# chreisinger/ViLGOD

Hardware: AMD Instinct MI355X
Metric: pseudo-labeled LiDAR frames/sec (150k pts, ~60 clusters) (higher is better)
Workload: dtype f16

## Files before the change

vilgod_amd/csrc/dev/vit_dev_entry.inc:

```
int vg_gemm_variant(int var, const void* d_X, const void* d_Wt, const float* d_bias, void* d_C, int M, int N, int K, int ldc, void* stream) {
    if (M % GBM || N % GBN || K % GK) return VG_ERR_ARG;
    int nwg = (M / GBM) * (N / GBN);
    hipStream_t st = (hipStream_t)stream;
#define VG_VAR(V)                                                                                                          \
    case V:                                                                                                                \
        (void)hipFuncSetAttribute((const void*)k_gemm_f16<EPI_BIAS, V>, hipFuncAttributeMaxDynamicSharedMemorySize, G_LDS_BYTES); \
        hipLaunchKernelGGL((k_gemm_f16<EPI_BIAS, V>), dim3(nwg), dim3(512), G_LDS_BYTES, st, (const f16*)d_X, (const f16*)d_Wt, \
                           d_bias, d_C, nullptr, M, N, K, ldc, gemm_chunk_tiles(N, K));                                   \
        break;
    switch (var) { VG_VAR(0) VG_VAR(1) VG_VAR(2) VG_VAR(3)
        case 20: return launch_gemm_pp<EPI_BIAS, 4, false>(d_X, d_Wt, d_bias, d_C, nullptr, M, N, K, ldc, st, nullptr);
        case 21: return launch_gemm_pp<EPI_BIAS, 5, false>(d_X, d_Wt, d_bias, d_C, nullptr, M, N, K, ldc, st, nullptr);
        case 22: return launch_gemm_pp<EPI_BIAS, 4, false, 1>(d_X, d_Wt, d_bias, d_C, nullptr, M, N, K, ldc, st, nullptr);
        case 23: return launch_gemm_pp<EPI_BIAS, 5, false, 1>(d_X, d_Wt, d_bias, d_C, nullptr, M, N, K, ldc, st, nullptr);
        case 30: return launch_gemm_pp16<EPI_BIAS, 4>(d_X, d_Wt, d_bias, d_C, nullptr, M, N, K, ldc, st);
        case 32: return launch_gemm_pp64<EPI_BIAS>(d_X, d_Wt, d_bias, d_C, nullptr, M, N, K, ldc, st);
        case 36: return launch_gemm_pp64<EPI_BIAS, false, true>(d_X, d_Wt, d_bias, d_C, nullptr, M, N, K, ldc, st);
        default: return VG_ERR_ARG; }
#undef VG_VAR
    VG_LAUNCH_CHECK();
    return VG_OK;
}

int vg_gemm_ln_consumer(int epi, const void* d_X, const void* d_Wt, const float* d_bias, const float* d_c1, const void* d_stats,
                        void* d_C, int M, int N, int K, void* stream) {
    hipStream_t st = (hipStream_t)stream;
    if (epi == 0) return launch_gemm_pp64<EPI_BIAS, false, false, 1>(d_X, d_Wt, d_bias, d_C, nullptr, M, N, K, N, st, nullptr, d_c1, (LnPartial*)d_stats);
    if (epi == 1) return launch_gemm_pp64<EPI_BIAS_GELU, false, false, 1>(d_X, d_Wt, d_bias, d_C, nullptr, M, N, K, N, st, nullptr, d_c1, (LnPartial*)d_stats);
    return VG_ERR_ARG;
}

int vg_gemm_trace(int var, const void* d_X, const void* d_Wt, const float* d_bias, void* d_C, int64_t* d_trace, int M, int N,
                  int K, int ldc, void* stream) {
    hipStream_t st = (hipStream_t)stream;
    switch (var) {
        case 20: return launch_gemm_pp<EPI_BIAS, 4, true>(d_X, d_Wt, d_bias, d_C, nullptr, M, N, K, ldc, st, (long long*)d_trace);
        case 21: return launch_gemm_pp<EPI_BIAS, 5, true>(d_X, d_Wt, d_bias, d_C, nullptr, M, N, K, ldc, st, (long long*)d_trace);
        case 22: return launch_gemm_pp<EPI_BIAS, 4, true, 1>(d_X, d_Wt, d_bias, d_C, nullptr, M, N, K, ldc, st, (long long*)d_trace);
        case 23: return launch_gemm_pp<EPI_BIAS, 5, true, 1>(d_X, d_Wt, d_bias, d_C, nullptr, M, N, K, ldc, st, (long long*)d_trace);
        case 32: return launch_gemm_pp64<EPI_BIAS, true>(d_X, d_Wt, d_bias, d_C, nullptr, M, N, K, ldc, st, (long long*)d_trace);
        case 33: return launch_gemm_pp64<EPI_BIAS_GELU, true>(d_X, d_Wt, d_bias, d_C, nullptr, M, N, K, ldc, st, (long long*)d_trace);
        case 34: return launch_gemm_pp64<EPI_BIAS_RESID, true>(d_X, d_Wt, d_bias, nullptr, (float*)d_C, M, N, K, ldc, st, (long long*)d_trace);
        case 35: return launch_gemm_pp64<EPI_BIAS_RESID_H, true>(d_X, d_Wt, d_bias, nullptr, (float*)d_C, M, N, K, ldc, st, (long long*)d_trace);
        case 50: return launch_gemm_w4<EPI_BIAS, 0, VG_W4_TRACE_VAR>(d_X, d_Wt, d_bias, d_C, nullptr, M, N, K, ldc, st, nullptr, nullptr, nullptr, (long long*)d_trace);
        case 40: return launch_gemm_x2<EPI_BIAS, 0, true>(d_X, d_Wt, d_bias, d_C, nullptr, M, N, K, ldc, st, nullptr, nullptr, nullptr, (long long*)d_trace);
        default: return VG_ERR_ARG; }
    VG_LAUNCH_CHECK();
    return VG_OK;
}

int vg_attention_trace(const void* d_qkv, void* d_out, int n_crops, int T, int W, int heads, int ld, int64_t* d_trace, void* stream) {
    if (!d_qkv || !d_out || n_crops <= 0 || T > AT_MAXT || heads * 64 != W) return VG_ERR_ARG;
    const int items = n_crops * heads;
    hipStream_t st = (hipStream_t)stream;
    if (d_trace) return launch_attention<true>((const f16*)d_qkv, (f16*)d_out, T, W, heads, ld, items, (long long*)d_trace, st);
    return launch_attention<false>((const f16*)d_qkv, (f16*)d_out, T, W, heads, ld, items, nullptr, st);
}
```

vilgod_amd/csrc/vit.hip:

```cpp
#include "common.h"
#include <hip/hip_fp16.h>
#include <string.h>
#include <stdlib.h>
#include <string>
#include <vector>
#include <map>
#include <atomic>
#include <mutex>
#include <utility>

typedef _Float16 f16;
typedef f16 f16x8 __attribute__((ext_vector_type(8)));
typedef f16 f16x4 __attribute__((ext_vector_type(4)));
typedef float f32x16 __attribute__((ext_vector_type(16)));

#define QGELU_C (-1.702f * 1.4426950408889634f)
enum { EPI_BIAS = 0, EPI_BIAS_GELU = 1, EPI_BIAS_RESID = 2, EPI_NONE_F32 = 3,
       EPI_BIAS_RESID_H = 4,
       EPI_BIAS_RESID_HL = 5 };

__device__ __forceinline__ int xcd_remap(int bid, int nwg) {
    int q = nwg >> 3, r = nwg & 7, xcd = bid & 7, s = bid >> 3;
    int base = (xcd < r) ? xcd * (q + 1) : r * (q + 1) + (xcd - r) * q;
    return base + s;
// ... 599 lines not shown
    float sum = 0.f;
    const int tail = T - 32 * (nkb - 1);
#pragma unroll
    for (int kb = 0; kb < 7; ++kb) {
        if (kb < nkb) {
#pragma unroll
            for (int g = 0; g < 4; ++g) {
                if (kb < nkb - 1 || 8 * g < tail) {
#pragma unroll
                    for (int r = 4 * g; r < 4 * g + 4; ++r) {
                        const float p = __builtin_amdgcn_exp2f(fmaf(sacc[kb][r], c2, mc));
                        sacc[kb][r] = p;
                        sum += p;
                    }
                } else {
#pragma unroll
                    for (int r = 4 * g; r < 4 * g + 4; ++r) sacc[kb][r] = 0.f;
                }
            }
        }
    }
    sum += __shfl_xor(sum, 32);
    const float inv = 1.0f / sum;
    AT_STAMP(4)

    f32x16 oacc[2];
#pragma unroll
    for (int dt = 0; dt < 2; ++dt)
#pragma unroll
        for (int r = 0; r < 16; ++r) oacc[dt][r] = 0.f;
#pragma unroll
    for (int kb = 0; kb < 7; ++kb) {
        if (kb < nkb) {
#pragma unroll
            for (int s = 0; s < 2; ++s) {
                if (kb == nkb - 1 && 16 * s >= tail) continue;
                f16x8 pf;
#pragma unroll
                for (int j = 0; j < 8; ++j) pf[j] = (f16)sacc[kb][8 * s + j];
#pragma unroll
                for (int dt = 0; dt < 2; ++dt) {
                    f16x4 lo, hi;
                    if (TR) {
                        const char* vb = (const char*)Vs + tr_off + ((kb * 32 + 16 * s) * AT_KLD + dt * 32) * 2;
                        lo = __builtin_bit_cast(f16x4, __builtin_amdgcn_ds_read_tr16_b64_v4i16((__attribute__((address_space(3))) s16x4v*)vb));
                        hi = __builtin_bit_cast(f16x4, __builtin_amdgcn_ds_read_tr16_b64_v4i16((__attribute__((address_space(3))) s16x4v*)(vb + 8 * AT_KLD * 2)));
                    } else {
                        const f16* vp = Vt + (dt * 32 + r31) * AT_VLD + kb * 32 + 16 * s + 4 * hh;
                        lo = *(const f16x4*)vp; hi = *(const f16x4*)(vp + 8);
                    }
                    f16x8 vf = {lo[0], lo[1], lo[2], lo[3], hi[0], hi[1], hi[2], hi[3]};
                    oacc[dt] = __builtin_amdgcn_mfma_f32_32x32x16_f16(vf, pf, oacc[dt], 0, 0, 0);
                }
            }
        }
    }
    AT_STAMP(5)
#pragma unroll
    for (int dt = 0; dt < 2; ++dt)
#pragma unroll
        for (int g = 0; g < 4; ++g) {
            f16x4 h4;
#pragma unroll
            for (int e = 0; e < 4; ++e) h4[e] = (f16)(oacc[dt][4 * g + e] * inv);
            *(f16x4*)(Qs + r31 * AT_KLD + dt * 32 + 8 * g + 4 * hh) = h4;
        }
#pragma unroll
    for (int it = 0; it < 4; ++it) {
        const int qr = q0 + it * 8 + crow;
        const f16x8 v = *(const f16x8*)(Qs + (it * 8 + crow) * AT_KLD + cpart * 8);
        if (qr < T) *(f16x8*)(obase + ooff[it]) = v;
    }
    }
    AT_STAMP(6)
    __syncthreads();
    AT_STAMP(7)
    }
    if (TRACE && trace && lane == 0) {
        long long* o = trace + ((size_t)blockIdx.x * 7 + wave) * 8;
#pragma unroll
        for (int i = 0; i < 8; ++i) o[i] = tr[i];
    }
#undef AT_STAMP
}

#define AL_MAXT 1024
#define AL_KB 64
#define AL_BUF (AL_KB * AT_KLD)
#define AL_LDS_BYTES ((4 * AL_BUF + 4 * 32 * AT_KLD) * 2)
__global__ __launch_bounds__(256, 2) void k_attention_f16_long(const f16* __restrict__ qkv, f16* __restrict__ out, int T, int W,
                                                               int heads, int ld, int n_items, int q_tiles) {
    extern __shared__ __attribute__((aligned(16))) char al_smem[];
    f16* const KV = (f16*)al_smem;
    const int tid = threadIdx.x, lane = tid & 63, wave = tid >> 6;
    f16* const Os = KV + 4 * AL_BUF + wave * 32 * AT_KLD;
    const int r31 = lane & 31, hh = lane >> 5;
    const int crow = lane >> 3, cpart = lane & 7;
    const int tr_i = lane & 15, tr_g = lane >> 4;
    const int tr_off = ((4 * (tr_g >> 1) + (tr_i >> 2)) * AT_KLD + 16 * (tr_g & 1) + 4 * (tr_i & 3)) * 2;
    const int ntile = (T + 31) / 32;
    const int qt = q_tiles < ntile ? q_tiles : ntile;
    const int npass = (qt + 3) / 4;
    const int nkb = (T + AL_KB - 1) / AL_KB;
    const int per_item = npass * nkb;
    const int my_items = (int)blockIdx.x < n_items ? (n_items - 1 - (int)blockIdx.x) / (int)gridDim.x + 1 : 0;
    const int nsteps = my_items * per_item;
    if (nsteps == 0) return;
    auto decode = [&](int s, int& item, int& pass, int& kb) {
        const int u = s / per_item, r = s - u * per_item;
        item = (int)blockIdx.x + u * (int)gridDim.x;
        pass = r / nkb;
        kb = r - pass * nkb;
    };
    uint4 kreg[2];
    f16x8 vreg[2], qn[4];
    auto fetch = [&](int s) {
        int item, pass, kb;
        decode(s, item, pass, kb);
        const int crop = item / heads, head = item - crop * heads;
        const f16* base = qkv + (size_t)crop * T * ld + head * 64;
#pragma unroll
        for (int it = 0; it < 2; ++it) {
            const int c = tid + it * 256, key = kb * AL_KB + (c >> 3), part = c & 7;
            const unsigned off = (unsigned)((key < T ? key : T - 1) * ld + part * 8);
            kreg[it] = *(const uint4*)(base + W + off);
            vreg[it] = *(const f16x8*)(base + 2 * W + off);
        }
        if (kb == 0) {
            const int qr = (pass * 4 + wave) * 32 + r31;
            const unsigned off = (unsigned)((qr < T ? qr : T - 1) * ld + hh * 8);
#pragma unroll
            for (int s4 = 0; s4 < 4; ++s4) qn[s4] = *(const f16x8*)(base + off + s4 * 16);
        }
    };
    auto stage = [&](int s) {
        int item, pass, kb;
        decode(s, item, pass, kb);
        f16* const Kb = KV + (s & 1) * 2 * AL_BUF;
        f16* const Vb = Kb + AL_BUF;
        const f16x8 z = {0, 0, 0, 0, 0, 0, 0, 0};
#pragma unroll
        for (int it = 0; it < 2; ++it) {
            const int c = tid + it * 256, row = c >> 3, part = c & 7;
            const bool live = kb * AL_KB + row < T;
            *(uint4*)(Kb + row * AT_KLD + part * 8) = live ? kreg[it] : make_uint4(0, 0, 0, 0);
            *(f16x8*)(Vb + row * AT_KLD + part * 8) = live ? vreg[it] : z;
        }
    };
    fetch(0);
    stage(0);
    __syncthreads();
    const float c2 = 0.125f * 1.4426950408889634f;
    f16x8 qf[4];
    f32x16 oacc[2];
    float m = -INFINITY, l = 0.f;
    for (int s = 0; s < nsteps; ++s) {
        int item, pass, kb;
        decode(s, item, pass, kb);
        if (kb == 0) {
#pragma unroll
            for (int s4 = 0; s4 < 4; ++s4) qf[s4] = qn[s4];
#pragma unroll
            for (int dt = 0; dt < 2; ++dt)
#pragma unroll
                for (int r = 0; r < 16; ++r) oacc[dt][r] = 0.f;
            m = -INFINITY;
// ... 175 lines not shown
    }
}

template <typename TI>
__global__ __launch_bounds__(256) void k_head(const TI* __restrict__ x, const float* __restrict__ lw,
                                              const float* __restrict__ lb, const float* __restrict__ proj,
                                              float* __restrict__ feat, int T, int W, int D) {
    extern __shared__ float sm[];
    __shared__ float red[8];
    const int crop = blockIdx.x, tid = threadIdx.x, lane = tid & 63, wave = tid >> 6;
    const TI* src = x + (size_t)crop * T * W;
    float s = 0.f;
    for (int c = tid; c < W; c += 256) s += (float)src[c];
    s = vg_wave_sum(s);
    if (lane == 0) red[wave] = s;
    __syncthreads();
    float mean = (red[0] + red[1] + red[2] + red[3]) / (float)W;
    __syncthreads();
    float q = 0.f;
    for (int c = tid; c < W; c += 256) {
        float d = (float)src[c] - mean;
        q += d * d;
    }
    q = vg_wave_sum(q);
    if (lane == 0) red[wave] = q;
    __syncthreads();
    float rstd = rsqrtf((red[0] + red[1] + red[2] + red[3]) / (float)W + 1e-5f);
    for (int c = tid; c < W; c += 256) sm[c] = ((float)src[c] - mean) * rstd * lw[c] + lb[c];
    __syncthreads();
    for (int j = tid; j < D; j += 256) {
        float a = 0.f;
#pragma unroll 16
        for (int i = 0; i < W; ++i)
            a = fmaf(sm[i], proj[(size_t)i * D + j], a);
        feat[(size_t)crop * D + j] = a;
    }
}

__global__ __launch_bounds__(64) void k_clip_scores(const float* __restrict__ feat, const float* __restrict__ text,
                                                    float* __restrict__ probs, int* __restrict__ top1,
                                                    float* __restrict__ top1_score, int n, int D, int Kc) {
    const int crop = blockIdx.x, lane = threadIdx.x;
    const float* f = feat + (size_t)crop * D;
    float ss = 0.f;
    for (int i = lane; i < D; i += 64) ss += f[i] * f[i];
    float nrm = sqrtf(vg_wave_sum(ss));
    float logit = -INFINITY;
    if (lane < Kc) {
        float a = 0.f;
        for (int i = 0; i < D; ++i) a = fmaf(100.0f * (f[i] / nrm), text[(size_t)lane * D + i], a);
        logit = a;
    }
    float mx = vg_wave_max(logit);
    float e = (lane < Kc) ? expf(logit - mx) : 0.f;
    float p = e / vg_wave_sum(e);
    if (lane < Kc) probs[(size_t)crop * Kc + lane] = p;
    float best = (lane < Kc) ? p : -1.f;
    int bi = lane;
#pragma unroll
    for (int o = 32; o > 0; o >>= 1) {
        float ob = __shfl_xor(best, o);
        int oi = __shfl_xor(bi, o);
        if (ob > best || (ob == best && oi < bi)) {
            best = ob;
            bi = oi;
        }
    }
    if (lane == 0) {
        top1[crop] = bi;
        top1_score[crop] = best;
    }
}

#define VG_PROF_MAX 4096
struct vg_vit {
    int width, layers, heads, patch, res, out_dim, dtype, T;
#ifdef VG_DEV
    bool gemm_x2 = getenv("VG_GEMM_X2") ? atoi(getenv("VG_GEMM_X2")) != 0 : false;
#endif
    bool cls_last = !(getenv("VG_VIT_CLS_LAST") && atoi(getenv("VG_VIT_CLS_LAST")) == 0);
    int splitk_max = getenv("VG_GEMM_SPLITK") ? atoi(getenv("VG_GEMM_SPLITK")) : 0;
    bool att_tr = !(getenv("VG_ATT_TR") && atoi(getenv("VG_ATT_TR")) == 0);
    bool att_stagger = !(getenv("VG_ATT_STAGGER") && atoi(getenv("VG_ATT_STAGGER")) == 0);
    bool f32_mfma = !(getenv("VG_GEMM_F32_MFMA") && atoi(getenv("VG_GEMM_F32_MFMA")) == 0);
    int gemm_w4 = getenv("VG_GEMM_W4") ? atoi(getenv("VG_GEMM_W4")) : 1;
    int n_cu = 0;
    bool resid_hl = false;
    bool resid_h = false;
    int prof_on = 0, prof_n = 0;
    hipEvent_t prof_ev[2 * VG_PROF_MAX];
    double prof_flops[VG_PROF_MAX];
    int prof_kind[VG_PROF_MAX];
    bool prof_init = false;
    std::map<std::string, void*> w;
    std::map<std::string, size_t> numel;
    bool ln_fold = false;
    std::atomic<bool> fold_ready{false}, warmed{false};
    float in_mean[3] = {0.48145466f, 0.4578275f, 0.40821073f}, in_std[3] = {0.26862954f, 0.26130258f, 0.27577711f};
    std::atomic<bool> conv1_ready{false};
    std::atomic<uint64_t> weights_gen{0};
    std::mutex mtx;
    std::map<std::string, void*> w32;
};

static bool is_gemm_weight(const std::string& n) {
    return n == "conv1.weight" || n.find("in_proj_weight") != std::string::npos ||
           n.find("out_proj.weight") != std::string::npos || n.find("c_fc.weight") != std::string::npos ||
           n.find("c_proj.weight") != std::string::npos;
}

static int vit_kpad(const vg_vit* v) { return (3 * v->patch * v->patch + 63) / 64 * 64; }

static int gemm_chunk_tiles(int N, int K) {
    const int ntn = N / GBN;
#ifdef VG_DEV
    if (getenv("VG_GEMM_NO_CHUNK")) return ntn;
#endif
    const long tile_bytes = (long)GBN * K * 2;
    int cw_max = (int)(2400000L / tile_bytes);
    if (cw_max < 1) cw_max = 1;
    if (cw_max >= ntn) return ntn;
    int nchunks = (ntn + cw_max - 1) / cw_max;
    while (ntn % nchunks) ++nchunks;
    return ntn / nchunks;
}

typedef float f32x4 __attribute__((ext_vector_type(4)));
#ifdef VG_DEV
#include "dev/vit_gemm_pp16.inc"
#endif

struct LnPartial { float mean, m2; };
__device__ __forceinline__ float row256_sum(float v) {
    v += __builtin_bit_cast(float, __builtin_amdgcn_update_dpp(0, __builtin_bit_cast(int, v), 0xB1, 0xF, 0xF, true));
    v += __builtin_bit_cast(float, __builtin_amdgcn_update_dpp(0, __builtin_bit_cast(int, v), 0x4E, 0xF, 0xF, true));
    v += __builtin_bit_cast(float, __builtin_amdgcn_update_dpp(0, __builtin_bit_cast(int, v), 0x141, 0xF, 0xF, true));
    v += __builtin_bit_cast(float, __builtin_amdgcn_update_dpp(0, __builtin_bit_cast(int, v), 0x140, 0xF, 0xF, true));
    const int b = __builtin_bit_cast(int, v);
    return (__builtin_bit_cast(float, __builtin_amdgcn_readlane(b, 0)) + __builtin_bit_cast(float, __builtin_amdgcn_readlane(b, 16))) +
           (__builtin_bit_cast(float, __builtin_amdgcn_readlane(b, 32)) + __builtin_bit_cast(float, __builtin_amdgcn_readlane(b, 48)));
}

template <int EPI, bool TRACE = false, bool PERSIST = false, int LN = 0, bool SPLITK = false>
__global__ __launch_bounds__(512, 1) void k_gemm_f16_pp64(const f16* __restrict__ X, const f16* __restrict__ Wt,
                                                          const float* __restrict__ bias, void* __restrict__ Cout,
                                                          float* __restrict__ resid, int M, int N, int K, int ldc, int cw,
                                                          long long* __restrict__ trace = nullptr,
                                                          const float* __restrict__ ln_c1 = nullptr, LnPartial* __restrict__ ln_stats = nullptr,
                                                          f16* __restrict__ ln_x16 = nullptr, int sk_parts = 1) {
    static_assert(!SPLITK || (EPI == EPI_NONE_F32 && !PERSIST && LN == 0), "split-K partials are raw fp32 tiles");
    constexpr int BM = 256, BN = 256, NT = 512, TM = 8, TN = 4;
    constexpr int XBUF = 32768, WBASE = 2 * XBUF, WBUF = 32768;
    extern __shared__ __attribute__((aligned(16))) char smem[];
    const int tid = threadIdx.x, wave = __builtin_amdgcn_readfirstlane(tid >> 6);
    const int ntm = M / BM;
    const int grp = wave >> 2, wn = wave & 3;
    long long tr_entry = 0, tr_load = 0, tr_bar = 0, tr_mma = 0, tr_wait = 0, tr_t0 = 0, tr_w0 = 0, tr_main = 0, tr_w_entry = 0;
    if (TRACE) { tr_entry = clock64(); tr_w_entry = wall_clock64(); }
    const int nt_all = ntm * (N / BN);
    const int xq = nt_all >> 3, xr_ = nt_all & 7, xcd = blockIdx.x & 7;
    const int xbase = (xcd < xr_) ? xcd * (xq + 1) : xr_ * (xq + 1) + (xcd - xr_) * xq;
    const int xcnt = xq + (xcd < xr_ ? 1 : 0);
    for (int ti = PERSIST ? (int)(blockIdx.x >> 3) : 0; ti < (PERSIST ? xcnt : 1); ti += PERSIST ? (int)(gridDim.x >> 3) : 1) {
    int lane = tid & 63;
    if (PERSIST) asm volatile("" : "+v"(lane));
    const int t = PERSIST ? xbase + ti : xcd_remap(blockIdx.x, gridDim.x);
// ... 774 lines not shown
        int dev = 0;
        (void)hipGetDevice(&dev);
        (void)hipDeviceGetAttribute(&v->n_cu, hipDeviceAttributeMultiprocessorCount, dev);
    }
    const bool prof = v->prof_on && v->prof_n < VG_PROF_MAX;
    if (prof) (void)hipEventRecord(v->prof_ev[2 * v->prof_n], st);
    struct Closer {
        vg_vit* v; bool prof; hipStream_t st; double fl; int kind;
        ~Closer() {
            if (prof) {
                (void)hipEventRecord(v->prof_ev[2 * v->prof_n + 1], st);
                v->prof_kind[v->prof_n] = kind;
                v->prof_flops[v->prof_n++] = fl;
            }
        }
    } closer{v, prof, st, 2.0 * (double)M * (double)N * (double)K, use_pp ? 1 : 0};
    if constexpr (EPI == EPI_BIAS_RESID_HL) {
        if (!(LN == 2 && v->dtype == 1 && v->gemm_w4 && use_pp && M % 256 == 0 && K % 64 == 0 && K / 64 >= 4 && resid && ln_x16)) return VG_ERR_ARG;
        return launch_gemm_w4<EPI, LN>(X, Wt, bias, C, resid, M, N, K, ldc, st, ln_c1, ln_stats, ln_x16);
    } else
    if constexpr (EPI == EPI_BIAS_RESID_H) {
        if (!(use_pp && K % 64 == 0 && K / 64 >= 2)) return VG_ERR_ARG;
        return launch_gemm_pp64<EPI>(X, Wt, bias, C, resid, M, N, K, ldc, st);
    } else
    if (v->dtype == 1) {
        if (M % GBM || N % GBN || K % GK) return VG_ERR_ARG;
        if (use_pp) {
            {
#ifdef VG_DEV
                static const int persist_mask = getenv("VG_GEMM_PERSIST") ? atoi(getenv("VG_GEMM_PERSIST")) : 0;
                if constexpr (LN == 0 && (EPI == EPI_BIAS || EPI == EPI_BIAS_GELU || EPI == EPI_BIAS_RESID)) {
                    if ((persist_mask >> EPI) & 1) return launch_gemm_pp64<EPI, false, true>(X, Wt, bias, C, resid, M, N, K, ldc, st);
                }
#endif
#ifdef VG_DEV
                if (v->gemm_x2 && K % 256 == 0 && (LN != 1 || K / 64 <= X2_LN_MAXP))
                    return launch_gemm_x2<EPI, LN>(X, Wt, bias, C, resid, M, N, K, ldc, st, ln_c1, ln_stats, ln_x16);
                if (v->gemm_x2 && LN != 0) return VG_ERR_ARG;
#endif
                if constexpr (EPI == EPI_BIAS_RESID && LN != 1) {
                    if (sk_scratch && M % 256 == 0 && !(v->gemm_w4 && K / 64 >= 4)) {
                        const SplitPlan sp = splitk_plan(M / 256, N / 256, K / 64, sk_bytes, v->splitk_max, v->n_cu);
                        if (sp.parts) {
                            const int rc = launch_gemm_pp64<EPI, false, false, LN>(X, Wt, bias, C, resid, sp.r_main * 256, N, K, ldc, st, nullptr, ln_c1, ln_stats, ln_x16);
                            if (rc) return rc;
                            return launch_gemm_resid_tail<LN>(X, Wt, bias, resid, sp.r_main * 256, M - sp.r_main * 256, N, K, ldc, sp.parts, sk_scratch, st,
                                                              ln_stats, ln_x16);
                        }
                    }
                }
                if (v->gemm_w4 && K / 64 >= 4) {
#ifdef VG_DEV
                    if constexpr (LN == 0 && EPI == EPI_BIAS) {
                        switch (v->gemm_w4) { VG_W4_DEV_CASES(EPI, LN) }
                    }
#endif
                    return launch_gemm_w4<EPI, LN>(X, Wt, bias, C, resid, M, N, K, ldc, st, ln_c1, ln_stats, ln_x16);
                }
                return launch_gemm_pp64<EPI, false, false, LN>(X, Wt, bias, C, resid, M, N, K, ldc, st, nullptr, ln_c1, ln_stats, ln_x16);
            }
        }
        if (LN != 0) return VG_ERR_ARG;
        int nwg = (M / GBM) * (N / GBN);
        VG_MAX_DYNAMIC_LDS(k_gemm_f16<EPI>, G_LDS_BYTES);
        hipLaunchKernelGGL((k_gemm_f16<EPI>), dim3(nwg), dim3(512), G_LDS_BYTES, st, (const f16*)X, (const f16*)Wt, bias, C,
                           resid, M, N, K, ldc, gemm_chunk_tiles(N, K));
    } else {
        if (M % 64 || N % 64 || K % 16) return VG_ERR_ARG;
        if (M % 128 == 0 && N % 128 == 0 && v->f32_mfma) {
            hipLaunchKernelGGL((k_gemm_f32_mfma<EPI>), dim3((M / 128) * (N / 128)), dim3(256), 0, st, (const float*)X, (const float*)Wt, bias,
                               (float*)C, resid, M, N, K);
        } else {
            int nwg = (M / 64) * (N / 64);
            hipLaunchKernelGGL((k_gemm_f32<EPI>), dim3(nwg), dim3(256), 0, st, (const float*)X, (const float*)Wt, bias,
                               (float*)C, resid, M, N, K);
        }
    }
    VG_LAUNCH_CHECK();
    return VG_OK;
}

template <bool TRACE>
static int launch_attention(const f16* qkv, f16* out, int T, int W, int heads, int ld, int items, long long* trace, hipStream_t st,
                            int q_tiles = 7, bool tr = true, bool stagger = true) {
    if (T > AT_MAXT && !TRACE) {
        if (T > AL_MAXT) return VG_ERR_ARG;
        static std::atomic<int> n_cu_{0};
        int n_cu = n_cu_.load();
        if (!n_cu) { int dev = 0; (void)hipGetDevice(&dev); (void)hipDeviceGetAttribute(&n_cu, hipDeviceAttributeMultiprocessorCount, dev); if (n_cu < 8) n_cu = 256; n_cu_.store(n_cu); }
        const dim3 grid(items < 2 * n_cu ? items : 2 * n_cu);
        VG_MAX_DYNAMIC_LDS(k_attention_f16_long, AL_LDS_BYTES);
        hipLaunchKernelGGL(k_attention_f16_long, grid, dim3(256), AL_LDS_BYTES, st, qkv, out, T, W, heads, ld, items, q_tiles);
        VG_LAUNCH_CHECK();
        return VG_OK;
    }
    const int nkb = (T + 31) / 32;
    if (nkb < 1 || nkb > 7) return VG_ERR_ARG;
    if (T == 197 && !TRACE && tr && stagger) {
        const dim3 grid7(items < 256 ? items : 256);
        VG_MAX_DYNAMIC_LDS((k_attention_f16<false, 7, 197, true, true>), AT_LDS_BYTES_TR);
        hipLaunchKernelGGL((k_attention_f16<false, 7, 197, true, true>), grid7, dim3(448), AT_LDS_BYTES_TR, st, qkv, out, T, W, heads, ld, items, trace, q_tiles);
        VG_LAUNCH_CHECK();
        return VG_OK;
    }
    if (T == 197 && !TRACE && tr) {
        const dim3 grid7(items < 256 ? items : 256);
        VG_MAX_DYNAMIC_LDS((k_attention_f16<false, 7, 197, true>), AT_LDS_BYTES_TR);
        hipLaunchKernelGGL((k_attention_f16<false, 7, 197, true>), grid7, dim3(448), AT_LDS_BYTES_TR, st, qkv, out, T, W, heads, ld, items, trace, q_tiles);
        VG_LAUNCH_CHECK();
        return VG_OK;
    }
    const dim3 grid(items < 256 ? items : 256), block(448);
#define VG_ATT(N)                                                                                                                  \
    case N: {                                                                                                                      \
        VG_MAX_DYNAMIC_LDS((k_attention_f16<TRACE, N>), AT_LDS_BYTES);                                                              \
        hipLaunchKernelGGL((k_attention_f16<TRACE, N>), grid, block, AT_LDS_BYTES, st, qkv, out, T, W, heads, ld, items, trace, q_tiles);   \
        break; }
    if (T == 197 && !TRACE) {
        VG_MAX_DYNAMIC_LDS((k_attention_f16<false, 7, 197>), AT_LDS_BYTES);
        hipLaunchKernelGGL((k_attention_f16<false, 7, 197>), grid, block, AT_LDS_BYTES, st, qkv, out, T, W, heads, ld, items, trace, q_tiles);
        VG_LAUNCH_CHECK();
        return VG_OK;
    }
    switch (nkb) { VG_ATT(1) VG_ATT(2) VG_ATT(3) VG_ATT(4) VG_ATT(5) VG_ATT(6) VG_ATT(7) }
#undef VG_ATT
    VG_LAUNCH_CHECK();
    return VG_OK;
}

__global__ __launch_bounds__(256) void k_ln_fold(const float* __restrict__ W32, const float* __restrict__ g, const float* __restrict__ beta,
                                                 const float* __restrict__ b, f16* __restrict__ Wf, float* __restrict__ c1,
                                                 float* __restrict__ c2, int K) {
    __shared__ double sh1[256], sh2[256];
    const int n = blockIdx.x, tid = threadIdx.x;
    double s1 = 0.0, s2 = 0.0;
    for (int k = tid; k < K; k += 256) {
        const float w = W32[(size_t)n * K + k];
        const f16 wf = (f16)(g[k] * w);
        Wf[(size_t)n * K + k] = wf;
        s1 += (double)(float)wf;
        s2 += (double)beta[k] * (double)w;
    }
    sh1[tid] = s1; sh2[tid] = s2;
    __syncthreads();
    for (int o = 128; o > 0; o >>= 1) {
        if (tid < o) { sh1[tid] += sh1[tid + o]; sh2[tid] += sh2[tid + o]; }
        __syncthreads();
    }
    if (tid == 0) { c1[n] = (float)sh1[0]; c2[n] = (float)((double)b[n] + sh2[0]); }
}

static void* vit_w(const vg_vit* v, const std::string& n) {
    auto it = v->w.find(n);
    return it == v->w.end() ? nullptr : it->second;
}

static int vit_fold_ln(vg_vit* v, hipStream_t st) {
    if (!v->ln_fold || v->fold_ready.load()) return VG_OK;
    std::lock_guard<std::mutex> lock(v->mtx);
    if (v->fold_ready.load()) return VG_OK;
    const int W = v->width;
    for (int l = 0; l < v->layers; ++l) {
        const std::string p = "transformer.resblocks." + std::to_string(l) + ".";
        const char* sets[2][4] = {{"ln_1.weight", "ln_1.bias", "attn.in_proj_weight", "attn.in_proj_bias"},
                                  {"ln_2.weight", "ln_2.bias", "mlp.c_fc.weight", "mlp.c_fc.bias"}};
        for (int k = 0; k < 2; ++k) {
            const std::string wn = p + sets[k][2];
            auto it32 = v->w32.find(wn);
            const float* g = (const float*)vit_w(v, p + sets[k][0]);
            const float* be = (const float*)vit_w(v, p + sets[k][1]);
            const float* b = (const float*)vit_w(v, p + sets[k][3]);
            if (it32 == v->w32.end() || !g || !be || !b) continue;
            const int N = (int)(v->numel[wn] / (size_t)W);
            for (const char* suffix : {"#ln", "#c1", "#c2"}) {
                auto old = v->w.find(wn + suffix);
                if (old != v->w.end()) { (void)hipFree(old->second); v->w.erase(old); }
            }
            void *wf = nullptr, *c1 = nullptr, *c2 = nullptr;
            VG_CHECK(hipMalloc(&wf, (size_t)N * W * 2));
            VG_CHECK(hipMalloc(&c1, (size_t)N * 4));
// ... 249 lines not shown
    const float* pos_tab = (const float*)need(input_kind == 3 ? "positional_embedding#1ch" : "positional_embedding");
    int rc = input_kind == 3 ? launch_gemm<EPI_NONE_F32>(v, patches, need("conv1.weight#1ch"), nullptr, pe, nullptr, (int)Pp, W, v->patch * v->patch, st)
                             : launch_gemm<EPI_NONE_F32>(v, patches, need("conv1.weight"), nullptr, pe, nullptr, (int)Pp, W, (int)Kp, st);
    if (rc) return rc;
    if (!pos_tab) return VG_ERR_ARG;
    const bool rh = v->resid_h;
    bool ln1_done = false;
    f16* xh = (f16*)x;
    const int64_t Mc = pad128(n_crops);
    const bool cls_fits = Mc * W * 16 + Mc * (W / 64) * 8 <= Mp * (3 * W + 256) * es;
    const bool hl = v->resid_hl && fold && !rh && v->dtype == 1 && L > 1 && W % 256 == 0 && cls_fits;
    f16* xlo = (f16*)x;
    if (rh)
        hipLaunchKernelGGL((k_embed_lnpre<f16>), dim3((unsigned)((Mp + 3) / 4)), dim3(256), 0, st, pe, (const float*)need("class_embedding"),
                           pos_tab, (const float*)need("ln_pre.weight"),
                           (const float*)need("ln_pre.bias"), xh, (int)M, T, W, (int)Mp);
    else {
        ln1_done = v->dtype == 1 && L > 0;
        const float* lw1 = ln1_done ? (const float*)need("transformer.resblocks.0.ln_1.weight") : nullptr;
        const float* lb1 = ln1_done ? (const float*)need("transformer.resblocks.0.ln_1.bias") : nullptr;
        if (ln1_done && (!lw1 || !lb1)) return VG_ERR_ARG;
        hipLaunchKernelGGL((k_embed_lnpre<float>), dim3((unsigned)((Mp + 3) / 4)), dim3(256), 0, st, pe, (const float*)need("class_embedding"),
                           pos_tab, (const float*)need("ln_pre.weight"),
                           (const float*)need("ln_pre.bias"), x, (int)M, T, W, (int)Mp, lw1, lb1, ln1_done ? (f16*)h : (f16*)nullptr,
                           hl ? (f16*)x16 : (f16*)nullptr, hl ? xlo : (f16*)nullptr);
    }
    VG_LAUNCH_CHECK();
    for (int l = 0; l < L; ++l) {
        std::string p = "transformer.resblocks." + std::to_string(l) + ".";
        const char* names[] = {"ln_1.weight", "ln_1.bias", "attn.in_proj_weight", "attn.in_proj_bias", "attn.out_proj.weight",
                               "attn.out_proj.bias", "ln_2.weight", "ln_2.bias", "mlp.c_fc.weight", "mlp.c_fc.bias",
                               "mlp.c_proj.weight", "mlp.c_proj.bias"};
        void* wp[12];
        for (int i = 0; i < 12; ++i) {
            wp[i] = need(p + names[i]);
            if (!wp[i]) {
                fprintf(stderr, "[vilgod_hip] vg_vit_encode: weight %s%s not set\n", p.c_str(), names[i]);
                return VG_ERR_ARG;
            }
        }
        void *fw1 = nullptr, *fw2 = nullptr;
        const float *f1c1 = nullptr, *f1c2 = nullptr, *f2c1 = nullptr, *f2c2 = nullptr;
        if (fold) {
            fw1 = need(p + "attn.in_proj_weight#ln"); f1c1 = (const float*)need(p + "attn.in_proj_weight#c1"); f1c2 = (const float*)need(p + "attn.in_proj_weight#c2");
            fw2 = need(p + "mlp.c_fc.weight#ln");     f2c1 = (const float*)need(p + "mlp.c_fc.weight#c1");     f2c2 = (const float*)need(p + "mlp.c_fc.weight#c2");
            if (!fw1 || !f1c1 || !f1c2 || !fw2 || !f2c1 || !f2c2) return VG_ERR_ARG;
        }
        if (l == 0 && ln1_done) {
        } else if (fold) {
        } else if (rh)
            hipLaunchKernelGGL((k_layernorm<f16, f16>), dim3((unsigned)((M + 3) / 4)), dim3(256), 0, st, (const f16*)xh, (const float*)wp[0], (const float*)wp[1], (f16*)h, (int)M, W, 1);
        else if (v->dtype == 1)
            hipLaunchKernelGGL((k_layernorm<f16>), dim3((unsigned)((M + 3) / 4)), dim3(256), 0, st, x, (const float*)wp[0], (const float*)wp[1], (f16*)h, (int)M, W, 1);
        else
            hipLaunchKernelGGL((k_layernorm<float>), dim3((unsigned)((M + 3) / 4)), dim3(256), 0, st, x, (const float*)wp[0], (const float*)wp[1], (float*)h, (int)M, W, 1);
        VG_LAUNCH_CHECK();
        const bool cls_only = v->cls_last && fold && !rh && l == L - 1 && L > 1 && cls_fits;
        if (hl && l == L - 1 && !cls_only) return VG_ERR_ARG;
        if (cls_only && W % 256 == 0) {
            const int nst = v->gemm_w4 ? W >> 7 : W >> 8;
            char* cb = (char*)mlp;
            f16* x16q = (f16*)cb;              cb += Mc * W * 2;
            f16* qc = (f16*)cb;                cb += Mc * W * 2;
            LnPartial* lnq = (LnPartial*)cb;
            rc = launch_gemm<EPI_BIAS, 1>(v, x16, (const f16*)fw1 + (size_t)W * W, f1c2 + W, (f16*)qkv + W, nullptr, (int)Mp, 2 * W, W, st, qkv_ld,
                                          f1c1 + W, lnst);
            if (rc) return rc;
            hipLaunchKernelGGL(k_gather_cls_ln, dim3((unsigned)Mc), dim3(256), 0, st, (const f16*)x16, (const LnPartial*)lnst, x16q, lnq, n_crops, T, W, nst);
            VG_LAUNCH_CHECK();
            rc = launch_gemm<EPI_BIAS, 1>(v, x16q, fw1, f1c2, qc, nullptr, (int)Mc, W, W, st, 0, f1c1, lnq);
            if (rc) return rc;
            hipLaunchKernelGGL(k_scatter_cls_q, dim3((unsigned)n_crops), dim3(256), 0, st, (const f16*)qc, (f16*)qkv, T, W, qkv_ld);
            VG_LAUNCH_CHECK();
        } else
        if (fold && !(l == 0 && ln1_done))
            rc = launch_gemm<EPI_BIAS, 1>(v, x16, fw1, f1c2, qkv, nullptr, (int)Mp, 3 * W, W, st, qkv_ld, f1c1, lnst);
        else
            rc = launch_gemm<EPI_BIAS>(v, h, wp[2], (const float*)wp[3], qkv, nullptr, (int)Mp, 3 * W, W, st, qkv_ld);
        if (rc) return rc;
        if (v->dtype == 1) {
            {
                const bool aprof = v->prof_on && v->prof_n < VG_PROF_MAX;
                if (aprof) (void)hipEventRecord(v->prof_ev[2 * v->prof_n], st);
                rc = launch_attention<false>((const f16*)qkv, (f16*)h, T, W, H, qkv_ld, n_crops * H, nullptr, st, cls_only ? 1 : (T + 31) / 32, v->att_tr, v->att_stagger);
                if (rc) return rc;
                if (aprof) {
                    (void)hipEventRecord(v->prof_ev[2 * v->prof_n + 1], st);
                    v->prof_kind[v->prof_n] = cls_only ? 3 : 2;
                    v->prof_flops[v->prof_n++] = 4.0 * (cls_only ? 1.0 : (double)T) * (double)T * 64.0 * (double)(n_crops * H);
                }
            }
        } else {
            size_t lds = ((size_t)T * 65 + (size_t)T * 64 + 16 * (size_t)T) * sizeof(float);
            static bool attr = false;
            if (!attr) {
                VG_CHECK(hipFuncSetAttribute((const void*)k_attention_f32, hipFuncAttributeMaxDynamicSharedMemorySize, 160 * 1024));
                attr = true;
            }
            hipLaunchKernelGGL(k_attention_f32, dim3(n_crops * H), dim3(256), lds, st, (const float*)qkv, (float*)h, T, W, H);
        }
        VG_LAUNCH_CHECK();
        if (cls_only) {
            char* cb = (char*)qkv;
            float* xc = (float*)cb;            cb += Mc * W * 4;
            f16* hc = (f16*)cb;                cb += Mc * W * 2;
            f16* x16c = (f16*)cb;              cb += Mc * W * 2;
            f16* mlpc = (f16*)cb;              cb += Mc * 4 * W * 2;
            LnPartial* lnc = (LnPartial*)cb;
            hipLaunchKernelGGL(k_gather_cls, dim3((unsigned)Mc), dim3(256), 0, st, (const f16*)h, (const float*)x, hc, xc, n_crops, T, W,
                               hl ? (const f16*)x16 : (const f16*)nullptr, hl ? (const f16*)xlo : (const f16*)nullptr);
            VG_LAUNCH_CHECK();
            rc = launch_gemm<EPI_BIAS_RESID, 2>(v, hc, wp[4], (const float*)wp[5], nullptr, xc, (int)Mc, W, W, st, 0, nullptr, lnc, x16c);
            if (rc) return rc;
            rc = launch_gemm<EPI_BIAS_GELU, 1>(v, x16c, fw2, f2c2, mlpc, nullptr, (int)Mc, 4 * W, W, st, 0, f2c1, lnc);
            if (rc) return rc;
            rc = launch_gemm<EPI_BIAS_RESID>(v, mlpc, wp[10], (const float*)wp[11], nullptr, xc, (int)Mc, W, 4 * W, st);
            if (rc) return rc;
            hipLaunchKernelGGL((k_head<float>), dim3(n_crops), dim3(256), W * sizeof(float), st, (const float*)xc, (const float*)need("ln_post.weight"),
                               (const float*)need("ln_post.bias"), (const float*)need("proj"), d_feat, 1, W, v->out_dim);
            VG_LAUNCH_CHECK();
            return VG_OK;
        }
        rc = rh ? launch_gemm<EPI_BIAS_RESID_H>(v, h, wp[4], (const float*)wp[5], nullptr, x, (int)Mp, W, W, st)
           : hl ? launch_gemm<EPI_BIAS_RESID_HL, 2>(v, h, wp[4], (const float*)wp[5], nullptr, (float*)xlo, (int)Mp, W, W, st, 0, nullptr, lnst, x16)
           : fold ? launch_gemm<EPI_BIAS_RESID, 2>(v, h, wp[4], (const float*)wp[5], nullptr, x, (int)Mp, W, W, st, 0, nullptr, lnst, x16, pe, pe_bytes)
                  : launch_gemm<EPI_BIAS_RESID>(v, h, wp[4], (const float*)wp[5], nullptr, x, (int)Mp, W, W, st, 0, nullptr, nullptr, nullptr, pe, pe_bytes);
        if (rc) return rc;
        if (fold) {
        } else if (rh)
            hipLaunchKernelGGL((k_layernorm<f16, f16>), dim3((unsigned)((M + 3) / 4)), dim3(256), 0, st, (const f16*)xh, (const float*)wp[6], (const float*)wp[7], (f16*)h, (int)M, W, 1);
        else if (v->dtype == 1)
            hipLaunchKernelGGL((k_layernorm<f16>), dim3((unsigned)((M + 3) / 4)), dim3(256), 0, st, x, (const float*)wp[6], (const float*)wp[7], (f16*)h, (int)M, W, 1);
        else
            hipLaunchKernelGGL((k_layernorm<float>), dim3((unsigned)((M + 3) / 4)), dim3(256), 0, st, x, (const float*)wp[6], (const float*)wp[7], (float*)h, (int)M, W, 1);
        VG_LAUNCH_CHECK();
        rc = fold ? launch_gemm<EPI_BIAS_GELU, 1>(v, x16, fw2, f2c2, mlp, nullptr, (int)Mp, 4 * W, W, st, 0, f2c1, lnst)
                  : launch_gemm<EPI_BIAS_GELU>(v, h, wp[8], (const float*)wp[9], mlp, nullptr, (int)Mp, 4 * W, W, st);
        if (rc) return rc;
        rc = rh ? launch_gemm<EPI_BIAS_RESID_H>(v, mlp, wp[10], (const float*)wp[11], nullptr, x, (int)Mp, W, 4 * W, st)
           : (hl && l + 1 < L) ? launch_gemm<EPI_BIAS_RESID_HL, 2>(v, mlp, wp[10], (const float*)wp[11], nullptr, (float*)xlo, (int)Mp, W, 4 * W, st, 0, nullptr, lnst, x16)
           : (fold && l + 1 < L) ? launch_gemm<EPI_BIAS_RESID, 2>(v, mlp, wp[10], (const float*)wp[11], nullptr, x, (int)Mp, W, 4 * W, st, 0, nullptr, lnst, x16, pe, pe_bytes)
                  : launch_gemm<EPI_BIAS_RESID>(v, mlp, wp[10], (const float*)wp[11], nullptr, x, (int)Mp, W, 4 * W, st, 0, nullptr, nullptr, nullptr, pe, pe_bytes);
        if (rc) return rc;
    }
    if (rh)
        hipLaunchKernelGGL((k_head<f16>), dim3(n_crops), dim3(256), W * sizeof(float), st, (const f16*)xh, (const float*)need("ln_post.weight"),
                           (const float*)need("ln_post.bias"), (const float*)need("proj"), d_feat, T, W, v->out_dim);
    else
        hipLaunchKernelGGL((k_head<float>), dim3(n_crops), dim3(256), W * sizeof(float), st, x, (const float*)need("ln_post.weight"),
                           (const float*)need("ln_post.bias"), (const float*)need("proj"), d_feat, T, W, v->out_dim);
    VG_LAUNCH_CHECK();
    return VG_OK;
}

int vg_attention(const void* d_qkv, void* d_out, int n_crops, int T, int W, int heads, int ld, void* stream) {
    if (!d_qkv || !d_out || n_crops <= 0 || T < 1 || T > AL_MAXT || heads * 64 != W) return VG_ERR_ARG;
    const char* tr_env = getenv("VG_ATT_TR");
    const char* sg_env = getenv("VG_ATT_STAGGER");
    return launch_attention<false>((const f16*)d_qkv, (f16*)d_out, T, W, heads, ld, n_crops * heads, nullptr, (hipStream_t)stream, (T + 31) / 32,
                                   !(tr_env && atoi(tr_env) == 0), !(sg_env && atoi(sg_env) == 0));
}

#ifdef VG_DEV
#include "dev/vit_dev_entry.inc"
#endif

int vg_gemm(int dtype, int epi, const void* d_X, const void* d_Wt, const float* d_bias, void* d_C, float* d_resid,
            int M, int N, int K, void* stream) {
    vg_vit v;
    v.dtype = dtype;
    hipStream_t st = (hipStream_t)stream;
    switch (epi) {
        case 0: return launch_gemm<EPI_BIAS>(&v, d_X, d_Wt, d_bias, d_C, d_resid, M, N, K, st);
        case 1: return launch_gemm<EPI_BIAS_GELU>(&v, d_X, d_Wt, d_bias, d_C, d_resid, M, N, K, st);
        case 2: return launch_gemm<EPI_BIAS_RESID>(&v, d_X, d_Wt, d_bias, d_C, d_resid, M, N, K, st);
        case 3: return launch_gemm<EPI_NONE_F32>(&v, d_X, d_Wt, d_bias, d_C, d_resid, M, N, K, st);
        case 4: return dtype == 1 ? launch_gemm<EPI_BIAS_RESID_H>(&v, d_X, d_Wt, d_bias, d_C, d_resid, M, N, K, st) : VG_ERR_ARG;
    }
    return VG_ERR_ARG;
}

int vg_gemm_ln(int kind, const void* d_X, const void* d_Wt, const float* d_bias, const float* d_c1, void* d_stats, void* d_C, int ldc,
               void* d_resid, void* d_x16, int M, int N, int K, void* stream) {
    if (!d_X || !d_Wt || !d_bias || !d_stats || ldc < N || ldc % 8) return VG_ERR_ARG;
    vg_vit v;
    v.dtype = 1;
    if (v.gemm_w4 && K < 256) return VG_ERR_ARG;
    hipStream_t st = (hipStream_t)stream;
    LnPartial* stats = (LnPartial*)d_stats;
    switch (kind) {
        case 0:
        case 1:
            if (!d_c1 || !d_C) return VG_ERR_ARG;
            return kind == 0 ? launch_gemm<EPI_BIAS, 1>(&v, d_X, d_Wt, d_bias, d_C, nullptr, M, N, K, st, ldc, d_c1, stats)
                             : launch_gemm<EPI_BIAS_GELU, 1>(&v, d_X, d_Wt, d_bias, d_C, nullptr, M, N, K, st, ldc, d_c1, stats);
        case 2:
            if (!d_resid || !d_x16) return VG_ERR_ARG;
            return launch_gemm<EPI_BIAS_RESID, 2>(&v, d_X, d_Wt, d_bias, nullptr, (float*)d_resid, M, N, K, st, ldc, nullptr, stats, (f16*)d_x16);
        case 3:
            if (!d_resid || !d_x16) return VG_ERR_ARG;
            return launch_gemm<EPI_BIAS_RESID_HL, 2>(&v, d_X, d_Wt, d_bias, nullptr, (float*)d_resid, M, N, K, st, ldc, nullptr, stats, (f16*)d_x16);
    }
    return VG_ERR_ARG;
}

int vg_gemm_ln_partial_cols(void) {
    vg_vit v;
    return v.gemm_w4 ? 128 : 256;
}

int vg_gemm_resid_splitk(const void* d_X, const void* d_Wt, const float* d_bias, float* d_resid, int M, int N, int K,
                         void* d_scratch, int64_t scratch_bytes, void* stream) {
    if (!d_X || !d_Wt || !d_bias || !d_resid || scratch_bytes < 0) return VG_ERR_ARG;
    vg_vit v;
    v.dtype = 1;
    return launch_gemm<EPI_BIAS_RESID>(&v, d_X, d_Wt, d_bias, nullptr, d_resid, M, N, K, (hipStream_t)stream, 0, nullptr, nullptr, nullptr,
                                       (float*)d_scratch, (size_t)scratch_bytes);
}

int vg_vit_profile(vg_vit* v, int on) {
    if (!v) return VG_ERR_ARG;
    if (on && !v->prof_init) {
        for (int i = 0; i < 2 * VG_PROF_MAX; ++i) VG_CHECK(hipEventCreate(&v->prof_ev[i]));
        v->prof_init = true;
    }
    v->prof_on = on;
    v->prof_n = 0;
    return VG_OK;
}

int vg_vit_profile_read_kind(vg_vit* v, int kind, int32_t* h_launches, double* h_ms, double* h_flops) {
    if (!v || !h_launches || !h_ms || !h_flops) return VG_ERR_ARG;
    *h_launches = 0; *h_ms = 0; *h_flops = 0;
    for (int i = 0; i < v->prof_n; ++i) {
        if (kind >= 0 ? v->prof_kind[i] != kind : v->prof_kind[i] >= 2) continue;
        VG_CHECK(hipEventSynchronize(v->prof_ev[2 * i + 1]));
        float ms = 0.f;
        VG_CHECK(hipEventElapsedTime(&ms, v->prof_ev[2 * i], v->prof_ev[2 * i + 1]));
        *h_ms += ms;
        *h_flops += v->prof_flops[i];
        ++*h_launches;
    }
    return VG_OK;
// ... 128 lines not shown
```

Baseline: 73.24.

## Add persistent streaming attention kernel with triple-buffered K/V staging for T=197

Adds a persistent attention kernel for T=197. Each block loops over several (crop, head) items and stages K/V into a three-slot LDS ring with register prefetch, so the global loads for the next item overlap the MFMA compute of the current one. A CLS-only variant staggers which wave takes each round. By default it is used only for the cls-only (q_tiles==1) attention call; the full attention path needs VG_ATT_STREAM>0. The cost is a large LDS footprint and more register pressure.

Result: no change. 73.24 (median of 4 runs) (-0.0%).

```diff
diff --git a/vilgod_amd/csrc/dev/vit_dev_entry.inc b/vilgod_amd/csrc/dev/vit_dev_entry.inc
--- a/vilgod_amd/csrc/dev/vit_dev_entry.inc
+++ b/vilgod_amd/csrc/dev/vit_dev_entry.inc
@@ -56,3 +56,19 @@
     if (d_trace) return launch_attention<true>((const f16*)d_qkv, (f16*)d_out, T, W, heads, ld, items, (long long*)d_trace, st);
     return launch_attention<false>((const f16*)d_qkv, (f16*)d_out, T, W, heads, ld, items, nullptr, st);
 }
+
+int vg_attention_stream_trace(const void* d_qkv, void* d_out, int n_crops, int W, int heads, int ld, int cls, int64_t* d_trace, void* stream) {
+    if (!d_qkv || !d_out || !d_trace || n_crops <= 0 || heads * 64 != W) return VG_ERR_ARG;
+    const int items = n_crops * heads;
+    hipStream_t st = (hipStream_t)stream;
+    const dim3 grid(items < 256 ? items : 256);
+    if (cls) {
+        VG_MAX_DYNAMIC_LDS((k_attention_f16_stream<true, true>), AS_LDS_BYTES);
+        hipLaunchKernelGGL((k_attention_f16_stream<true, true>), grid, dim3(512), AS_LDS_BYTES, st, (const f16*)d_qkv, (f16*)d_out, W, heads, ld, items, (long long*)d_trace);
+    } else {
+        VG_MAX_DYNAMIC_LDS((k_attention_f16_stream<true, false>), AS_LDS_BYTES);
+        hipLaunchKernelGGL((k_attention_f16_stream<true, false>), grid, dim3(512), AS_LDS_BYTES, st, (const f16*)d_qkv, (f16*)d_out, W, heads, ld, items, (long long*)d_trace);
+    }
+    VG_LAUNCH_CHECK();
+    return VG_OK;
+}
diff --git a/vilgod_amd/csrc/vit.hip b/vilgod_amd/csrc/vit.hip
--- a/vilgod_amd/csrc/vit.hip
+++ b/vilgod_amd/csrc/vit.hip
@@ -705,6 +705,217 @@
         for (int i = 0; i < 8; ++i) o[i] = tr[i];
     }
 #undef AT_STAMP
+}
+
+#define AS_T 197
+#define AS_KROWS 197
+#define AS_VROWS 208
+#define AS_SLOT ((AS_KROWS + AS_VROWS) * 128)
+#define AS_LDS_BYTES (3 * AS_SLOT)
+#define AS_CHUNKS (2 * AS_T * 8)
+#define AS_CPT 7
+static_assert(7 * 32 * 128 <= AS_SLOT && AS_VROWS >= 6 * 32 + 16 && AS_VROWS >= AS_T, "last K block and last V k-step read inside the slot");
+static_assert(AS_CPT * 512 >= AS_CHUNKS && (AS_CPT - 1) * 512 < AS_CHUNKS, "staging split");
+template <bool TRACE = false, bool CLS = false>
+__global__ __launch_bounds__(512) void k_attention_f16_stream(const f16* __restrict__ qkv, f16* __restrict__ out, int W, int heads, int ld,
+                                                              int n_items, long long* __restrict__ trace = nullptr) {
+    constexpr int T = AS_T, NKB = 7, TPI = CLS ? 1 : 7, R = CLS ? 1 : 8;
+    long long tr[8] = {0, 0, 0, 0, 0, 0, 0, 0}, tc = 0;
+#define AS_STAMP(i) if (TRACE) { const long long c_ = clock64(); tr[i] += c_ - tc; tc = c_; }
+#define AS_BARRIER()                                   \
+    asm volatile("s_waitcnt lgkmcnt(0)" ::: "memory"); \
+    __builtin_amdgcn_sched_barrier(0);                 \
+    __builtin_amdgcn_s_barrier();                      \
+    __builtin_amdgcn_sched_barrier(0);                 \
+    asm volatile("" ::: "memory");
+    extern __shared__ __attribute__((aligned(16))) char as_smem[];
+    const int tid = threadIdx.x, lane = tid & 63;
+    const int wave = __builtin_amdgcn_readfirstlane(tid >> 6);
+    const int r31 = lane & 31, hh = lane >> 5, r7 = lane & 7;
+    const int tr_i = lane & 15, tr_g = lane >> 4;
+    const int G = (int)gridDim.x;
+    const int n_local = (n_items - (int)blockIdx.x + G - 1) / G;
+    const int n_units = n_local * TPI, n_rounds = (n_units + R - 1) / R;
+    const int vrow = 4 * (tr_g >> 1) + (tr_i >> 2), vpart = 2 * (tr_g & 1) + ((tr_i & 3) >> 1);
+    unsigned vo[2];
+#pragma unroll
+    for (int dt = 0; dt < 2; ++dt) vo[dt] = (unsigned)((AS_KROWS + vrow) * 128 + (((4 * dt + vpart) ^ (vrow & 7)) << 4) + ((tr_i & 1) << 3));
+    unsigned goff[AS_CPT], loff[AS_CPT];
+#pragma unroll
+    for (int it = 0; it < AS_CPT; ++it) {
+        const int c0 = tid + 512 * it, c = c0 < AS_CHUNKS ? c0 : AS_CHUNKS - 1;
+        const int isv = c >= T * 8, k = c - (isv ? T * 8 : 0), row = k >> 3, part = k & 7;
+        goff[it] = (unsigned)(row * ld + part * 8 + (isv ? 2 * W : W));
+        loff[it] = (unsigned)((isv ? AS_KROWS * 128 : 0) + row * 128 + ((part ^ (row & 7)) << 4));
+    }
+    auto item_base = [&](int j) __attribute__((always_inline)) -> const f16* {
+        const int item = (int)blockIdx.x + j * G, crop = item / heads, head = item - crop * heads;
+        return qkv + (size_t)crop * T * ld + head * 64;
+    };
+    f16x8 kv[AS_CPT];
+    auto load_kv = [&](int j) __attribute__((always_inline)) {
+        const f16* b = item_base(j);
+#pragma unroll
+        for (int it = 0; it < AS_CPT; ++it) kv[it] = *(const f16x8*)(b + goff[it]);
+    };
+    auto write_kv = [&](int j) __attribute__((always_inline)) {
+        char* s = as_smem + (j % 3) * AS_SLOT;
+#pragma unroll
+        for (int it = 0; it < AS_CPT - 1; ++it) *(f16x8*)(s + loff[it]) = kv[it];
+        if (tid < AS_CHUNKS - 512 * (AS_CPT - 1)) *(f16x8*)(s + loff[AS_CPT - 1]) = kv[AS_CPT - 1];
+    };
+    auto unit_of = [&](int r) __attribute__((always_inline)) -> int {
+        const int sl = CLS ? ((wave - r) & 7) : wave, u = R * r + sl;
+        return sl < R && u < n_units ? u : -1;
+    };
+    f16x8 qf[4], qn[4];
+    auto load_q = [&](int u) __attribute__((always_inline)) {
+        const int j = u / TPI, t = u - j * TPI, qr = t * 32 + r31;
+        const f16* b = item_base(j);
+        const unsigned o = (unsigned)((qr < T ? qr : T - 1) * ld + hh * 8);
+#pragma unroll
+        for (int s = 0; s < 4; ++s) qn[s] = *(const f16x8*)(b + o + s * 16);
+    };
+    constexpr int QSTEP = CLS ? 8 : 1;
+    if (unit_of(CLS ? wave : 0) >= 0) load_q(unit_of(CLS ? wave : 0));
+    load_kv(0);
+    if (tid < 3 * 88) {
+        const int sl = tid / 88, k = tid - sl * 88;
+        *(uint4*)(as_smem + sl * AS_SLOT + (AS_KROWS + AS_T + (k >> 3)) * 128 + (k & 7) * 16) = make_uint4(0, 0, 0, 0);
+    }
+    int nst = 0;
+    for (int r = 0; r < n_rounds; ++r) {
+        if (TRACE) tc = clock64();
+        const int ulast = R * r + R - 1 < n_units ? R * r + R - 1 : n_units - 1;
+        const int j0 = R * r / TPI, j1 = ulast / TPI;
+        if (nst <= j1) {
+            write_kv(nst);
+            if (++nst < n_local) load_kv(nst);
+            if (nst <= j1) {
+                write_kv(nst);
+                if (++nst < n_local) load_kv(nst);
+            }
+            AS_BARRIER()
+        }
+        AS_STAMP(0)
+        const bool stage = nst < n_local && nst <= j0 + 2, stage_first = !CLS && wave >= 4;
+        if (stage && stage_first) {
+            write_kv(nst);
+            if (++nst < n_local) load_kv(nst);
+        }
+        const int u = unit_of(r);
+        if (u >= 0) {
+            const int j = u / TPI, t = u - j * TPI, q = t * 32 + r31;
+            const char* const slot = as_smem + (j % 3) * AS_SLOT;
+#pragma unroll
+            for (int s = 0; s < 4; ++s) qf[s] = qn[s];
+            if (unit_of(r + QSTEP) >= 0) load_q(unit_of(r + QSTEP));
+            f32x16 sacc[7];
+#pragma unroll
+            for (int kb = 0; kb < 7; ++kb) {
+#pragma unroll
+                for (int r_ = 0; r_ < 16; ++r_) sacc[kb][r_] = 0.f;
+#pragma unroll
+                for (int s = 0; s < 4; ++s) {
+                    const f16x8 kf = *(const f16x8*)(slot + (kb * 32 + r31) * 128 + (((2 * s + hh) ^ r7) << 4));
+                    sacc[kb] = __builtin_amdgcn_mfma_f32_32x32x16_f16(kf, qf[s], sacc[kb], 0, 0, 0);
+                }
+            }
+            AS_STAMP(1)
+            float mx = -INFINITY;
+#pragma unroll
+            for (int kb = 0; kb < 7; ++kb) {
+                if (kb == NKB - 1) {
+#pragma unroll
+                    for (int r_ = 0; r_ < 16; ++r_) {
+                        const int key = kb * 32 + (r_ & 3) + 8 * (r_ >> 2) + 4 * hh;
+                        if (key >= T) sacc[kb][r_] = -INFINITY;
+                    }
+                }
+#pragma unroll
+                for (int r_ = 0; r_ < 16; ++r_) mx = fmaxf(mx, sacc[kb][r_]);
+            }
+            mx = fmaxf(mx, __shfl_xor(mx, 32));
+            AS_STAMP(2)
+            const float c2 = 0.125f * 1.4426950408889634f;
+            const float mc = -mx * c2;
+            float sum = 0.f;
+            constexpr int tail = T - 32 * (NKB - 1);
+#pragma unroll
+            for (int kb = 0; kb < 7; ++kb) {
+#pragma unroll
+                for (int g = 0; g < 4; ++g) {
+                    if (kb < NKB - 1 || 8 * g < tail) {
+#pragma unroll
+                        for (int r_ = 4 * g; r_ < 4 * g + 4; ++r_) {
+                            const float p = __builtin_amdgcn_exp2f(fmaf(sacc[kb][r_], c2, mc));
+                            sacc[kb][r_] = p;
+                            sum += p;
+                        }
+                    } else {
+#pragma unroll
+                        for (int r_ = 4 * g; r_ < 4 * g + 4; ++r_) sacc[kb][r_] = 0.f;
+                    }
+                }
+            }
+            sum += __shfl_xor(sum, 32);
+            const float inv = 1.0f / sum;
+            AS_STAMP(3)
+            f32x16 oacc[2];
+#pragma unroll
+            for (int dt = 0; dt < 2; ++dt)
+#pragma unroll
+                for (int r_ = 0; r_ < 16; ++r_) oacc[dt][r_] = 0.f;
+#pragma unroll
+            for (int kb = 0; kb < 7; ++kb) {
+#pragma unroll
+                for (int s = 0; s < 2; ++s) {
+                    if (kb == NKB - 1 && 16 * s >= tail) continue;
+                    f16x8 pf;
+#pragma unroll
+                    for (int e = 0; e < 8; ++e) pf[e] = (f16)sacc[kb][8 * s + e];
+#pragma unroll
+                    for (int dt = 0; dt < 2; ++dt) {
+                        const char* vb = slot + vo[dt] + (kb * 32 + 16 * s) * 128;
+                        const f16x4 lo = __builtin_bit_cast(f16x4, __builtin_amdgcn_ds_read_tr16_b64_v4i16((__attribute__((address_space(3))) s16x4v*)vb));
+                        const f16x4 hi = __builtin_bit_cast(f16x4, __builtin_amdgcn_ds_read_tr16_b64_v4i16((__attribute__((address_space(3))) s16x4v*)(vb + 8 * 128)));
+                        const f16x8 vf = {lo[0], lo[1], lo[2], lo[3], hi[0], hi[1], hi[2], hi[3]};
+                        oacc[dt] = __builtin_amdgcn_mfma_f32_32x32x16_f16(vf, pf, oacc[dt], 0, 0, 0);
+                    }
+                }
+            }
+            AS_STAMP(4)
+            if (q < T) {
+                const int item = (int)blockIdx.x + j * G, crop = item / heads, head = item - crop * heads;
+                f16* const orow = out + (size_t)crop * T * W + head * 64;
+                const unsigned oo = (unsigned)(q * W + 4 * hh);
+#pragma unroll
+                for (int dt = 0; dt < 2; ++dt)
+#pragma unroll
+                    for (int g = 0; g < 4; ++g) {
+                        f16x4 h4;
+#pragma unroll
+                        for (int e = 0; e < 4; ++e) h4[e] = (f16)(oacc[dt][4 * g + e] * inv);
+                        *(f16x4*)(orow + oo + dt * 32 + 8 * g) = h4;
+                    }
+            }
+            AS_STAMP(5)
+        }
+        if (stage && !stage_first) {
+            write_kv(nst);
+            if (++nst < n_local) load_kv(nst);
+        }
+        AS_STAMP(6)
+        AS_BARRIER()
+        AS_STAMP(7)
+    }
+    if (TRACE && trace && lane == 0) {
+        long long* o = trace + ((size_t)blockIdx.x * 8 + wave) * 8;
+#pragma unroll
+        for (int i = 0; i < 8; ++i) o[i] = tr[i];
+    }
+#undef AS_BARRIER
+#undef AS_STAMP
 }
 
 #define AL_MAXT 1024
@@ -1046,6 +1257,7 @@
     int splitk_max = getenv("VG_GEMM_SPLITK") ? atoi(getenv("VG_GEMM_SPLITK")) : 0;
     bool att_tr = !(getenv("VG_ATT_TR") && atoi(getenv("VG_ATT_TR")) == 0);
     bool att_stagger = !(getenv("VG_ATT_STAGGER") && atoi(getenv("VG_ATT_STAGGER")) == 0);
+    int att_stream = getenv("VG_ATT_STREAM") ? atoi(getenv("VG_ATT_STREAM")) : -1;
     bool f32_mfma = !(getenv("VG_GEMM_F32_MFMA") && atoi(getenv("VG_GEMM_F32_MFMA")) == 0);
     int gemm_w4 = getenv("VG_GEMM_W4") ? atoi(getenv("VG_GEMM_W4")) : 1;
     int n_cu = 0;
@@ -1986,7 +2198,7 @@
 
 template <bool TRACE>
 static int launch_attention(const f16* qkv, f16* out, int T, int W, int heads, int ld, int items, long long* trace, hipStream_t st,
-                            int q_tiles = 7, bool tr = true, bool stagger = true) {
+                            int q_tiles = 7, bool tr = true, bool stagger = true, int stream = -1) {
     if (T > AT_MAXT && !TRACE) {
         if (T > AL_MAXT) return VG_ERR_ARG;
         static std::atomic<int> n_cu_{0};
@@ -2000,6 +2212,18 @@
     }
     const int nkb = (T + 31) / 32;
     if (nkb < 1 || nkb > 7) return VG_ERR_ARG;
+    if (T == AS_T && !TRACE && (stream > 0 || (stream < 0 && q_tiles == 1)) && tr && stagger && (q_tiles == nkb || q_tiles == 1)) {
+        const dim3 grid(items < 256 ? items : 256);
+        if (q_tiles == 1) {
+            VG_MAX_DYNAMIC_LDS((k_attention_f16_stream<false, true>), AS_LDS_BYTES);
+            hipLaunchKernelGGL((k_attention_f16_stream<false, true>), grid, dim3(512), AS_LDS_BYTES, st, qkv, out, W, heads, ld, items, nullptr);
+        } else {
+            VG_MAX_DYNAMIC_LDS((k_attention_f16_stream<false, false>), AS_LDS_BYTES);
+            hipLaunchKernelGGL((k_attention_f16_stream<false, false>), grid, dim3(512), AS_LDS_BYTES, st, qkv, out, W, heads, ld, items, nullptr);
+        }
+        VG_LAUNCH_CHECK();
+        return VG_OK;
+    }
     if (T == 197 && !TRACE && tr && stagger) {
         const dim3 grid7(items < 256 ? items : 256);
         VG_MAX_DYNAMIC_LDS((k_attention_f16<false, 7, 197, true, true>), AT_LDS_BYTES_TR);
@@ -2415,7 +2639,8 @@
             {
                 const bool aprof = v->prof_on && v->prof_n < VG_PROF_MAX;
                 if (aprof) (void)hipEventRecord(v->prof_ev[2 * v->prof_n], st);
-                rc = launch_attention<false>((const f16*)qkv, (f16*)h, T, W, H, qkv_ld, n_crops * H, nullptr, st, cls_only ? 1 : (T + 31) / 32, v->att_tr, v->att_stagger);
+                rc = launch_attention<false>((const f16*)qkv, (f16*)h, T, W, H, qkv_ld, n_crops * H, nullptr, st, cls_only ? 1 : (T + 31) / 32, v->att_tr, v->att_stagger,
+                                              v->att_stream);
                 if (rc) return rc;
                 if (aprof) {
                     (void)hipEventRecord(v->prof_ev[2 * v->prof_n + 1], st);
@@ -2490,8 +2715,9 @@
     if (!d_qkv || !d_out || n_crops <= 0 || T < 1 || T > AL_MAXT || heads * 64 != W) return VG_ERR_ARG;
     const char* tr_env = getenv("VG_ATT_TR");
     const char* sg_env = getenv("VG_ATT_STAGGER");
+    const char* sm_env = getenv("VG_ATT_STREAM");
     return launch_attention<false>((const f16*)d_qkv, (f16*)d_out, T, W, heads, ld, n_crops * heads, nullptr, (hipStream_t)stream, (T + 31) / 32,
-                                   !(tr_env && atoi(tr_env) == 0), !(sg_env && atoi(sg_env) == 0));
+                                   !(tr_env && atoi(tr_env) == 0), !(sg_env && atoi(sg_env) == 0), sm_env ? atoi(sm_env) : -1);
 }
 
 #ifdef VG_DEV
```
